# zama-ai/concrete-ntt

Measured on AMD Instinct MI355X. Metric: forward+inverse NTTs/sec (prime64, N=1024, batched) per GPU; % HBM roofline, higher is better.
Workload: dtype u64; 1 GPU; prime64 N=1024 p=4611686018427322369 batch=65536 per GPU: fwd + mul_assign_normalize (pre-transformed rhs) + inv, device-resident, fused in one kernel (cntt_prime64_mul_ntt_batch); polynomial_size=1024, batch_per_gpu=65536, modulus=4611686018427322369, launcher=single process, rccl_ranks=0

## Files before the change

concrete-ntt_amd/csrc/host_core.hip:

```cpp
#include <atomic>
#include <cstdarg>
#include <cstdio>
#include <string>

#include "aux_kernels.hpp"
#include "host_common.hpp"

static thread_local std::string g_err;

int fail(int code, const char *fmt, ...) {
    char buf[512];
    va_list ap;
    va_start(ap, fmt);
    vsnprintf(buf, sizeof buf, fmt, ap);
    va_end(ap);
    g_err = buf;
    return code;
}

extern "C" const char *cntt_last_error(void) { return g_err.c_str(); }
#include "build_hash.inc"
extern "C" const char *cntt_version(void) { return "cntt-hip 0.3 (gfx950) csrc:" CNTT_CSRC_HASH; }
extern "C" int cntt_device_count(void) {
    int n = 0;
    if (hipGetDeviceCount(&n) != hipSuccess) return 0;
    return n;
}

namespace {
struct SwitchDef { const char *name; int dflt; };
constexpr SwitchDef kSwitches[DBG_COUNT] = {
    {"fp", 1}, {"pm64", 1}, {"blk", 1}, {"mul32_blk", 1}, {"ext32_blk", 1}, {"ext_one", 1}, {"ext_split", -1}, {"native_acc", 1},
    {"product_fused", -1}, {"plan52_via32", 1}, {"native_ext", 1}, {"native_gadget", 0}};
std::atomic<int> g_switch[DBG_COUNT] = {{1}, {1}, {1}, {1}, {1}, {1}, {-1}, {1}, {-1}, {1}, {1}, {0}};
int switch_index(const char *key) {
    if (!key) return -1;
    for (int i = 0; i < (int)DBG_COUNT; ++i)
        if (std::strcmp(key, kSwitches[i].name) == 0) return i;
    return -1;
}
}
int cntt::debug_switch(DebugSwitch key) { return g_switch[key].load(std::memory_order_relaxed); }
extern "C" int cntt_debug_set(const char *key, int value) {
    if (key && std::strcmp(key, "reset") == 0) {
        for (int i = 0; i < (int)DBG_COUNT; ++i) g_switch[i].store(kSwitches[i].dflt);
        return CNTT_OK;
    }
    const int i = switch_index(key);
    if (i < 0) return fail(CNTT_EINVAL, "cntt_debug_set: unknown switch '%s'", key ? key : "(null)");
    if (value < -1 || value > 1) return fail(CNTT_EINVAL, "cntt_debug_set: %s takes -1 (library default), 0 or 1", key);
    g_switch[i].store(value < 0 ? kSwitches[i].dflt : value);
    return CNTT_OK;
}
extern "C" int cntt_debug_get(const char *key, int *value) {
    const int i = switch_index(key);
    if (i < 0 || !value) return fail(CNTT_EINVAL, "cntt_debug_get: unknown switch '%s'", key ? key : "(null)");
    *value = g_switch[i].load();
    return CNTT_OK;
}

extern "C" int cntt_shard_bounds(size_t batch, int world, int rank, size_t *begin, size_t *end) {
    if (world < 1 || rank < 0 || rank >= world || !begin || !end) return fail(CNTT_EINVAL, "cntt_shard_bounds: need 0 <= rank < world and non-NULL outputs");
    const size_t base = batch / (size_t)world, rem = batch % (size_t)world, r = (size_t)rank;
    *begin = r * base + (r < rem ? r : rem);
    *end = *begin + base + (r < rem ? 1 : 0);
    return CNTT_OK;
}

extern "C" unsigned cntt_ew_grid(size_t work_items) { return ew_grid(work_items); }

extern "C" int cntt_fill_uniform_u64(uint64_t *dst, size_t count, uint64_t bound, uint64_t seed, void *st) {
    if (!dst && count) return fail(CNTT_EINVAL, "dst is NULL");
    if (!count) return CNTT_OK;
    hipLaunchKernelGGL((fill_uniform_kernel<uint64_t>), dim3(ew_grid(count)), dim3(256), 0, (hipStream_t)st, dst, count,
                       bound, seed);
    HIP_TRY(hipGetLastError());
    return CNTT_OK;
}
extern "C" int cntt_fill_uniform_u32(uint32_t *dst, size_t count, uint32_t bound, uint64_t seed, void *st) {
    if (!dst && count) return fail(CNTT_EINVAL, "dst is NULL");
    if (!count) return CNTT_OK;
    hipLaunchKernelGGL((fill_uniform_kernel<uint32_t>), dim3(ew_grid(count)), dim3(256), 0, (hipStream_t)st, dst, count,
                       bound, seed);
    HIP_TRY(hipGetLastError());
    return CNTT_OK;
}
```

concrete-ntt_amd/csrc/ntt_launch.hpp:

```cpp
#pragma once
#include <hip/hip_runtime.h>
#include <stdint.h>

#include "ntt_arith.hpp"

namespace cntt {
enum DebugSwitch : int {
    DBG_FP = 0,
    DBG_PM64,
    DBG_BLK,
    DBG_MUL32_BLK,
    DBG_EXT32_BLK,
    DBG_EXT_ONE,
    DBG_EXT_SPLIT,
    DBG_NATIVE_ACC,
    DBG_PRODUCT_FUSED,
    DBG_PLAN52_VIA32,
    DBG_NATIVE_EXT,
    DBG_NATIVE_GADGET,
    DBG_COUNT
};
int debug_switch(DebugSwitch key);
}

namespace cntt {

template <class T> struct MaxLdsLogN;
template <> struct MaxLdsLogN<uint64_t> { static constexpr int value = 14; };
template <> struct MaxLdsLogN<uint32_t> { static constexpr int value = 15; };
constexpr int MAX_FPW_LOGN = 15;
template <class T> struct MinLogN;
template <> struct MinLogN<uint64_t> { static constexpr int value = 4; };
template <> struct MinLogN<uint32_t> { static constexpr int value = 5; };

template <class T, bool INV>
hipError_t launch_ntt(int logn, int cls, T *data, const TwPair<T> *tw, const ModParams<T> &P, uint32_t nsub,
                      uint32_t depth, hipStream_t stream);

template <int CLS>
hipError_t launch_ntt_fp(int logn, bool inv, uint64_t *data, const TwPair<uint64_t> *tw, const ModParams<uint64_t> &P,
                         uint32_t nsub, hipStream_t stream);
template <int CLS>
hipError_t launch_mul_ntt_fp(int logn, uint64_t *lhs, const uint64_t *rhs_ntt, const TwPair<uint64_t> *twf,
                             const TwPair<uint64_t> *twi, const ModParams<uint64_t> &P, uint32_t nsub, hipStream_t stream);

template <class T>
hipError_t launch_mul_ntt(int logn, int cls, T *lhs, const T *rhs_ntt, const TwPair<T> *twf, const TwPair<T> *twi,
                          const ModParams<T> &P, uint32_t nsub, hipStream_t stream);

template <class T, int NOUT>
hipError_t launch_ext_ntt_n(int logn, int cls, T *out, const T *terms, const T *key_ntt, const TwPair<T> *twf,
                            const TwPair<T> *twi, const ModParams<T> &P, uint32_t batch, uint32_t nterms, bool accumulate,
                            hipStream_t stream, uint32_t ostride);
bool ext_split_enabled();
template <class T>
inline hipError_t launch_ext_ntt(int logn, int cls, T *out, const T *terms, const T *key_ntt, const TwPair<T> *twf,
                                 const TwPair<T> *twi, const ModParams<T> &P, uint32_t batch, uint32_t nterms, uint32_t nout,
                                 bool accumulate, hipStream_t stream) {
    hipError_t e = hipErrorNotSupported;
    switch (nout) {
    case 0: return hipSuccess;
    case 1: e = launch_ext_ntt_n<T, 1>(logn, cls, out, terms, key_ntt, twf, twi, P, batch, nterms, accumulate, stream, 1); break;
    case 2: e = launch_ext_ntt_n<T, 2>(logn, cls, out, terms, key_ntt, twf, twi, P, batch, nterms, accumulate, stream, 2); break;
    case 3: e = launch_ext_ntt_n<T, 3>(logn, cls, out, terms, key_ntt, twf, twi, P, batch, nterms, accumulate, stream, 3); break;
    case 4: e = launch_ext_ntt_n<T, 4>(logn, cls, out, terms, key_ntt, twf, twi, P, batch, nterms, accumulate, stream, 4); break;
    default: return hipErrorNotSupported;
    }
    if (e != hipErrorNotSupported || nout < 3 || !ext_split_enabled()) return e;
    (void)hipGetLastError();
    e = launch_ext_ntt_n<T, 2>(logn, cls, out, terms, key_ntt, twf, twi, P, batch, nterms, accumulate, stream, nout);
    if (e != hipSuccess) return e;
    T *out2 = out + ((size_t)2 << logn);
    const T *key2 = key_ntt + ((size_t)2 << logn);
    if (nout == 3) return launch_ext_ntt_n<T, 1>(logn, cls, out2, terms, key2, twf, twi, P, batch, nterms, accumulate, stream, nout);
    return launch_ext_ntt_n<T, 2>(logn, cls, out2, terms, key2, twf, twi, P, batch, nterms, accumulate, stream, nout);
}

struct SplitArgs;
struct CrtArgs;
struct AccArgs;
struct ProductArgs;
hipError_t launch_product_fused2(int logn, int cls, bool inv, uint64_t *standard, uint32_t *res32, const void *tables,
                                 const ProductArgs &A, uint32_t batch, bool flag, hipStream_t st);
template <int KIND>
hipError_t launch_native_fused(int logn, void *prod, const void *lhs, const void *rhs, const void *tables, const SplitArgs &S,
                               const CrtArgs &C, uint32_t batch, uint32_t *scratch, hipStream_t st, const AccArgs *acc,
                               const void *tables_acc);
constexpr bool native_fused_acc(int kind, int logn) {
    return kind == 2 ? (logn >= 5 && logn <= 13) : kind == 5 ? (logn >= 5 && logn <= 12) : (kind >= 0 && kind <= 4 && logn >= 5 && logn <= 14);
}
bool native_acc_enabled();
struct KeyPlanes;
constexpr int NATIVE_EXT_MAX_LOGN = 12;
template <int KIND>
hipError_t launch_native_ext(int logn, void *out, const void *terms, const KeyPlanes &K, const void *tables_acc, const SplitArgs &S,
                             const AccArgs &C, uint32_t batch, uint32_t nterms, uint32_t nout, bool accumulate, hipStream_t st);
struct GadgetCall {
    const void *polys;
    const uint32_t *rot;
    const void *addend;
    uint64_t off;
    uint32_t npolys, levels, base_log;
    uint32_t cmux;
    uint32_t add_out;
};
template <int KIND>
hipError_t launch_native_ext_gadget(int logn, void *out, const GadgetCall &G, const KeyPlanes &K, const void *tables_acc,
                                    const SplitArgs &S, const AccArgs &C, uint32_t batch, uint32_t nout, hipStream_t st);
inline int device_num_cus() {
    int dev = 0, n = 0;
    if (hipGetDevice(&dev) != hipSuccess) return 256;
    if (hipDeviceGetAttribute(&n, hipDeviceAttributeMultiprocessorCount, dev) != hipSuccess || n <= 0) n = 256;
    return n;
}
constexpr bool native_fused_lds13(int kind) { return kind == 0 || kind == 1 || kind == 4; }
inline bool native_fused_persistent(int kind, int logn) {
    if (native_fused_acc(kind, logn) && native_acc_enabled()) return false;
    return (logn == 13 && !native_fused_lds13(kind)) || logn == 14 || logn == 15 || (kind == 2 && logn >= 5 && logn <= 12);
}
inline size_t native_fused_tile_words(int logn) { return logn < 12 ? (size_t)4096 : (size_t)1 << logn; }
inline uint32_t native_fused_grid(int logn, int ncu, uint32_t batch) {
    const size_t ppb = native_fused_tile_words(logn) >> logn;
    const size_t groups = ((size_t)batch + ppb - 1) / ppb, g = (size_t)ncu * (logn >= 14 ? 1u : logn == 13 ? 2u : 4u);
    return (uint32_t)(g < groups ? g : groups);
}
inline size_t native_fused_scratch_words(int kind, int logn, int nprimes, int ncu, uint32_t batch) {
    if (!native_fused_persistent(kind, logn)) return 0;
    return (size_t)native_fused_grid(logn, ncu, batch) * (size_t)(nprimes - 1) * native_fused_tile_words(logn);
}

}
```

concrete-ntt_amd/csrc/ntt_mul_inst.inc:

```
#include "ntt_mul_one.hpp"

namespace cntt {

template <class T, int LOGN>
static hipError_t mul_logn(int logn, int cls, T *lhs, const T *rhs, const TwPair<T> *twf, const TwPair<T> *twi,
                           const ModParams<T> &P, uint32_t nsub, hipStream_t stream) {
    if constexpr (sizeof(T) == 4 && LOGN >= 13 && LOGN <= 15) {
        if (logn == LOGN) {
            if constexpr (LOGN >= 14) {
                if (mul32_blk_enabled()) {
                    if constexpr (mul32_blk_wins(LOGN, CLS_FPW)) {
                        if (cls == CLS_FPW) return mul32_blk_one<T, LOGN, CLS_FPW>(lhs, rhs, twf, twi, P, nsub, stream);
                    }
                    if constexpr (mul32_blk_wins(LOGN, CLS_LAZY)) {
                        if (cls == CLS_LAZY) return mul32_blk_one<T, LOGN, CLS_LAZY>(lhs, rhs, twf, twi, P, nsub, stream);
                    }
                    if constexpr (mul32_blk_wins(LOGN, CLS_STRICT)) {
                        if (cls == CLS_STRICT) return mul32_blk_one<T, LOGN, CLS_STRICT>(lhs, rhs, twf, twi, P, nsub, stream);
                    }
                }
            }
            if constexpr (LOGN <= MAX_FPW_LOGN) {
                if (cls == CLS_FPW) {
                    hipLaunchKernelGGL((mul_kernel_one<T, LOGN, CLS_FPW>), dim3(nsub), dim3(MulOne<T, LOGN, CLS_FPW>::TPP), 0, stream, lhs,
                                       rhs, twf, twi, P);
                    return hipGetLastError();
                }
            }
            switch (cls) {
            case CLS_LAZY:
                hipLaunchKernelGGL((mul_kernel_one<T, LOGN, CLS_LAZY>), dim3(nsub), dim3(MulOne<T, LOGN, CLS_LAZY>::TPP), 0, stream, lhs, rhs,
                                   twf, twi, P);
                break;
            case CLS_STRICT:
                hipLaunchKernelGGL((mul_kernel_one<T, LOGN, CLS_STRICT>), dim3(nsub), dim3(MulOne<T, LOGN, CLS_STRICT>::TPP), 0, stream, lhs,
                                   rhs, twf, twi, P);
                break;
            case CLS_GENERIC:
                hipLaunchKernelGGL((mul_kernel_one<T, LOGN, CLS_GENERIC>), dim3(nsub), dim3(MulOne<T, LOGN, CLS_GENERIC>::TPP), 0, stream, lhs,
                                   rhs, twf, twi, P);
                break;
            default: return hipErrorNotSupported;
            }
            return hipGetLastError();
        }
        return mul_logn<T, LOGN + 1>(logn, cls, lhs, rhs, twf, twi, P, nsub, stream);
    } else if constexpr (LOGN > 14) {
        if constexpr (sizeof(T) == 8 && LOGN == 15) {
            if (logn != 15) return hipErrorNotSupported;
            if (cls == CLS_FP) return launch_mul_ntt_fp<CLS_FP>(15, lhs, rhs, twf, twi, P, nsub, stream);
            if (cls == CLS_FP51) return launch_mul_ntt_fp<CLS_FP51>(15, lhs, rhs, twf, twi, P, nsub, stream);
            if (cls == CLS_PM64) return launch_mul_ntt_fp<CLS_PM64>(15, lhs, rhs, twf, twi, P, nsub, stream);
            if (cls == CLS_LAZY) return mul_32k_one<T, CLS_LAZY>(lhs, rhs, twf, twi, P, nsub, stream);
            if (cls == CLS_STRICT) return mul_32k_one<T, CLS_STRICT>(lhs, rhs, twf, twi, P, nsub, stream);
        }
        return hipErrorNotSupported;
    } else {
        using K0 = NttKernel<T, LOGN, false, CLS_LAZY, false>;
        if (logn == LOGN) {
            if constexpr (mul_blk_eligible((int)sizeof(T), LOGN, CLS_LAZY)) {
                if (cls == CLS_FP) return launch_mul_ntt_fp<CLS_FP>(LOGN, lhs, rhs, twf, twi, P, nsub, stream);
                if (cls == CLS_FP51) return launch_mul_ntt_fp<CLS_FP51>(LOGN, lhs, rhs, twf, twi, P, nsub, stream);
                if (cls == CLS_PM64) return launch_mul_ntt_fp<CLS_PM64>(LOGN, lhs, rhs, twf, twi, P, nsub, stream);
                if (cls == CLS_LAZY) return mul_blk_one<T, LOGN, CLS_LAZY>(lhs, rhs, twf, twi, P, nsub, stream);
                if (cls == CLS_STRICT) return mul_blk_one<T, LOGN, CLS_STRICT>(lhs, rhs, twf, twi, P, nsub, stream);
                return hipErrorNotSupported;
            }
            if constexpr (K0::NPASS > 1 && K0::TPP <= 256 && (size_t)K0::IMG_ENTRIES * sizeof(TwPair<T>) <= 32768) {
                if constexpr (sizeof(T) == 8) {
                    if (cls == CLS_FP) return launch_mul_ntt_fp<CLS_FP>(LOGN, lhs, rhs, twf, twi, P, nsub, stream);
                    if (cls == CLS_FP51) return launch_mul_ntt_fp<CLS_FP51>(LOGN, lhs, rhs, twf, twi, P, nsub, stream);
                    if (cls == CLS_PM64) return launch_mul_ntt_fp<CLS_PM64>(LOGN, lhs, rhs, twf, twi, P, nsub, stream);
                }
                if constexpr (sizeof(T) == 4) {
                    if (cls == CLS_FPW) return mul_one<T, LOGN, CLS_FPW>(lhs, rhs, twf, twi, P, nsub, stream);
                }
                switch (cls) {
                case CLS_LAZY: return mul_one<T, LOGN, CLS_LAZY>(lhs, rhs, twf, twi, P, nsub, stream);
                case CLS_STRICT: return mul_one<T, LOGN, CLS_STRICT>(lhs, rhs, twf, twi, P, nsub, stream);
                default: return mul_one<T, LOGN, CLS_GENERIC>(lhs, rhs, twf, twi, P, nsub, stream);
                }
            } else {
                return hipErrorNotSupported;
            }
        }
        return mul_logn<T, LOGN + 1>(logn, cls, lhs, rhs, twf, twi, P, nsub, stream);
    }
}

template <>
hipError_t launch_mul_ntt<INST_T>(int logn, int cls, INST_T *lhs, const INST_T *rhs_ntt, const TwPair<INST_T> *twf,
                                  const TwPair<INST_T> *twi, const ModParams<INST_T> &P, uint32_t nsub,
                                  hipStream_t stream) {
    if (nsub == 0) return hipSuccess;
    if (logn < MinLogN<INST_T>::value || logn > 15) return hipErrorNotSupported;
    return mul_logn<INST_T, MinLogN<INST_T>::value>(logn, cls, lhs, rhs_ntt, twf, twi, P, nsub, stream);
}

}
```

concrete-ntt_amd/csrc/ntt_mul_one.hpp:

```cpp
#pragma once
#include <cstdlib>
#include "ntt_blk.hpp"
#include "ntt_kernel.hpp"
#include "ntt_launch.hpp"

namespace cntt {

template <class T, int LOGN> struct MulShape {
    using K0 = NttKernel<T, LOGN, false, CLS_LAZY, false>;
    static constexpr size_t IMG = (size_t)K0::IMG_ENTRIES * sizeof(TwPair<T>);
    static constexpr size_t LDS_MAX = 160 * 1024;
    static constexpr size_t lds(int block) { return (size_t)(block / K0::TPP) * K0::LDS_WORDS_1 * sizeof(T) + 2 * IMG; }
    static constexpr bool THREE_SMALL = 3 * lds(256) <= LDS_MAX && K0::E == 16;
    static constexpr bool ONE_BIG = !THREE_SMALL && lds(768) <= LDS_MAX && K0::E == 16 && K0::TPP <= 256 && 768 % K0::TPP == 0;
    static constexpr bool TWO_SMALL = 2 * lds(256) <= LDS_MAX;
    static constexpr int BLOCK = THREE_SMALL ? 256 : ONE_BIG ? 768 : TWO_SMALL ? 256 : 512;
    static constexpr int PER_CU = THREE_SMALL ? 3 : ONE_BIG ? 1 : TWO_SMALL ? 2 : 1;
    static constexpr int WAVES_PER_SIMD = BLOCK / 64 * PER_CU / 4;
    static_assert(lds(BLOCK) * PER_CU <= LDS_MAX, "fused product kernel does not fit LDS");
};

static int mul_num_cus() {
    int dev = 0, n = 0;
    if (hipGetDevice(&dev) != hipSuccess) return 256;
    if (hipDeviceGetAttribute(&n, hipDeviceAttributeMultiprocessorCount, dev) != hipSuccess || n <= 0) n = 256;
    return n;
}

template <class T, int LOGN, int CLS>
static hipError_t mul_one(T *lhs, const T *rhs, const TwPair<T> *twf, const TwPair<T> *twi, const ModParams<T> &P,
                          uint32_t nsub, hipStream_t stream) {
    using SH = MulShape<T, LOGN>;
    using K = MulWp<T, LOGN, CLS, SH::BLOCK>;
    const uint32_t ntiles = (nsub + K::PPB - 1) / K::PPB;
    uint32_t grid = (uint32_t)mul_num_cus() * SH::PER_CU;
    if (grid > ntiles) grid = ntiles;
    hipLaunchKernelGGL((mul_kernel_wp<T, LOGN, CLS, SH::BLOCK, SH::WAVES_PER_SIMD>), dim3(grid), dim3(SH::BLOCK), 0, stream,
                       lhs, rhs, twf, twi, P, nsub);
    return hipGetLastError();
}

constexpr bool mul_blk_eligible(int bytes, int logn, int cls) { return bytes == 8 && logn >= 12 && logn <= 14 && cls != CLS_GENERIC; }
template <int LOGN, int CLS> struct MulBlkShape {
    static constexpr int WPW = 4;
    static constexpr int PER_CU = LOGN == 12 ? 4 : LOGN == 13 ? 2 : 1;
    static constexpr bool PREFETCH = true;
    static constexpr int TWC = 2;
};
template <class T, int LOGN, int CLS>
static hipError_t mul_blk_one(T *lhs, const T *rhs, const TwPair<T> *twf, const TwPair<T> *twi, const ModParams<T> &P,
                              uint32_t nsub, hipStream_t stream) {
    using SH = MulBlkShape<LOGN, CLS>;
    using K = MulBlk<T, LOGN, CLS, SH::TWC, SH::PREFETCH>;
    uint32_t grid = (uint32_t)mul_num_cus() * SH::PER_CU;
    if (grid > nsub) grid = nsub;
    hipLaunchKernelGGL((mul_kernel_blk<T, LOGN, CLS, SH::WPW, SH::TWC, SH::PREFETCH>), dim3(grid), dim3(K::WPB), 0, stream, lhs, rhs,
                       twf, twi, P, nsub);
    return hipGetLastError();
}

constexpr bool mul32_blk_wins(int logn, int cls) {
    return (cls == CLS_LAZY && (logn == 14 || logn == 15)) || (cls == CLS_STRICT && logn == 15) || (cls == CLS_FPW && logn == 14);
}
static bool mul32_blk_enabled() { return debug_switch(DBG_MUL32_BLK) != 0; }
template <class T, int LOGN, int CLS>
static hipError_t mul32_blk_one(T *lhs, const T *rhs, const TwPair<T> *twf, const TwPair<T> *twi, const ModParams<T> &P,
                                uint32_t nsub, hipStream_t stream) {
    constexpr bool PF = LOGN == 14 && CLS == CLS_LAZY;
    using K = MulBlk<T, LOGN, CLS, 2, PF>;
    uint32_t grid = (uint32_t)mul_num_cus() * (LOGN == 14 ? 2 : 1);
    if (grid > nsub) grid = nsub;
    hipLaunchKernelGGL((mul_kernel_blk<T, LOGN, CLS, 4, 2, PF>), dim3(grid), dim3(K::WPB), 0, stream, lhs, rhs, twf, twi, P, nsub);
    return hipGetLastError();
}

template <class T, int CLS>
static hipError_t mul_32k_one(T *lhs, const T *rhs, const TwPair<T> *twf, const TwPair<T> *twi, const ModParams<T> &P,
                              uint32_t nsub, hipStream_t stream) {
    uint32_t grid = (uint32_t)mul_num_cus();
    if (grid > nsub) grid = nsub;
    hipLaunchKernelGGL((mul_kernel_32k<T, CLS, 4>), dim3(grid), dim3(Mul32k<T, CLS>::WPB), 0, stream, lhs, rhs, twf, twi, P, nsub);
    return hipGetLastError();
}

}
```

Baseline: 239.8 million NTT/s.

## Add paired-polynomial wavefront kernel for fused N=1024 multiply NTT

Adds a new fused forward-multiply-inverse kernel for 64-bit lazy-class N=1024 in which each wavefront transforms two polynomials at once. Twiddle loads, stage bookkeeping and the per-wave LDS buffer are shared across the pair. The next tile's two polynomials are prefetched asynchronously while the current tile is computed. The kernel is enabled by default through a new mul_pair switch. In exchange it doubles register pressure per thread and serialises the LDS transposes for the two polynomials, which may lower occupancy.

```diff
diff --git a/concrete-ntt_amd/csrc/host_core.hip b/concrete-ntt_amd/csrc/host_core.hip
--- a/concrete-ntt_amd/csrc/host_core.hip
+++ b/concrete-ntt_amd/csrc/host_core.hip
@@ -31,8 +31,8 @@
 struct SwitchDef { const char *name; int dflt; };
 constexpr SwitchDef kSwitches[DBG_COUNT] = {
     {"fp", 1}, {"pm64", 1}, {"blk", 1}, {"mul32_blk", 1}, {"ext32_blk", 1}, {"ext_one", 1}, {"ext_split", -1}, {"native_acc", 1},
-    {"product_fused", -1}, {"plan52_via32", 1}, {"native_ext", 1}, {"native_gadget", 0}};
-std::atomic<int> g_switch[DBG_COUNT] = {{1}, {1}, {1}, {1}, {1}, {1}, {-1}, {1}, {-1}, {1}, {1}, {0}};
+    {"product_fused", -1}, {"plan52_via32", 1}, {"native_ext", 1}, {"native_gadget", 0}, {"mul_pair", 1}};
+std::atomic<int> g_switch[DBG_COUNT] = {{1}, {1}, {1}, {1}, {1}, {1}, {-1}, {1}, {-1}, {1}, {1}, {0}, {1}};
 int switch_index(const char *key) {
     if (!key) return -1;
     for (int i = 0; i < (int)DBG_COUNT; ++i)
diff --git a/concrete-ntt_amd/csrc/ntt_launch.hpp b/concrete-ntt_amd/csrc/ntt_launch.hpp
--- a/concrete-ntt_amd/csrc/ntt_launch.hpp
+++ b/concrete-ntt_amd/csrc/ntt_launch.hpp
@@ -18,6 +18,7 @@
     DBG_PLAN52_VIA32,
     DBG_NATIVE_EXT,
     DBG_NATIVE_GADGET,
+    DBG_MUL_PAIR,
     DBG_COUNT
 };
 int debug_switch(DebugSwitch key);
diff --git a/concrete-ntt_amd/csrc/ntt_mul_inst.inc b/concrete-ntt_amd/csrc/ntt_mul_inst.inc
--- a/concrete-ntt_amd/csrc/ntt_mul_inst.inc
+++ b/concrete-ntt_amd/csrc/ntt_mul_inst.inc
@@ -75,6 +75,9 @@
                 if constexpr (sizeof(T) == 4) {
                     if (cls == CLS_FPW) return mul_one<T, LOGN, CLS_FPW>(lhs, rhs, twf, twi, P, nsub, stream);
                 }
+                if constexpr (mul_pair_eligible((int)sizeof(T), LOGN, CLS_LAZY)) {
+                    if (cls == CLS_LAZY && mul_pair_enabled()) return mul_pair_one<T, LOGN, CLS_LAZY>(lhs, rhs, twf, twi, P, nsub, stream);
+                }
                 switch (cls) {
                 case CLS_LAZY: return mul_one<T, LOGN, CLS_LAZY>(lhs, rhs, twf, twi, P, nsub, stream);
                 case CLS_STRICT: return mul_one<T, LOGN, CLS_STRICT>(lhs, rhs, twf, twi, P, nsub, stream);
diff --git a/concrete-ntt_amd/csrc/ntt_mul_one.hpp b/concrete-ntt_amd/csrc/ntt_mul_one.hpp
--- a/concrete-ntt_amd/csrc/ntt_mul_one.hpp
+++ b/concrete-ntt_amd/csrc/ntt_mul_one.hpp
@@ -3,6 +3,7 @@
 #include "ntt_blk.hpp"
 #include "ntt_kernel.hpp"
 #include "ntt_launch.hpp"
+#include "ntt_mul_pair.hpp"
 
 namespace cntt {
 
@@ -37,6 +38,23 @@
     if (grid > ntiles) grid = ntiles;
     hipLaunchKernelGGL((mul_kernel_wp<T, LOGN, CLS, SH::BLOCK, SH::WAVES_PER_SIMD>), dim3(grid), dim3(SH::BLOCK), 0, stream,
                        lhs, rhs, twf, twi, P, nsub);
+    return hipGetLastError();
+}
+
+constexpr bool mul_pair_eligible(int bytes, int logn, int cls) { return bytes == 8 && logn == 10 && cls == CLS_LAZY; }
+static bool mul_pair_enabled() { return debug_switch(DBG_MUL_PAIR) != 0; }
+template <class T, int LOGN, int CLS>
+static hipError_t mul_pair_one(T *lhs, const T *rhs, const TwPair<T> *twf, const TwPair<T> *twi, const ModParams<T> &P,
+                               uint32_t nsub, hipStream_t stream) {
+    constexpr int BLOCK = 256, PER_CU = 2, WAVES_PER_SIMD = BLOCK / 64 * PER_CU / 4;
+    using K = MulWpPair<T, LOGN, CLS, BLOCK>;
+    static_assert(PER_CU * ((size_t)(BLOCK / K::TPP) * K::FB::LDS_WORDS_1 * sizeof(T) + 2 * MulShape<T, LOGN>::IMG) <= MulShape<T, LOGN>::LDS_MAX,
+                  "pair kernel does not fit LDS");
+    const uint32_t ntiles = (nsub + K::PPB - 1) / K::PPB;
+    uint32_t grid = (uint32_t)mul_num_cus() * PER_CU;
+    if (grid > ntiles) grid = ntiles;
+    hipLaunchKernelGGL((mul_kernel_wp_pair<T, LOGN, CLS, BLOCK, WAVES_PER_SIMD>), dim3(grid), dim3(BLOCK), 0, stream, lhs, rhs, twf, twi,
+                       P, nsub);
     return hipGetLastError();
 }
 
diff --git a/concrete-ntt_amd/csrc/ntt_mul_pair.hpp b/concrete-ntt_amd/csrc/ntt_mul_pair.hpp
--- /dev/null
+++ b/concrete-ntt_amd/csrc/ntt_mul_pair.hpp
@@ -0,0 +1,200 @@
+#pragma once
+#include "ntt_kernel.hpp"
+
+namespace cntt {
+
+template <class T, int LOGN, int CLS, int WPB>
+struct MulWpPair {
+    using F = NttWp<T, LOGN, false, CLS, WPB>;
+    using I = NttWp<T, LOGN, true, CLS, WPB>;
+    using FB = typename F::B;
+    using IB = typename I::B;
+    template <bool INV> using KB = std::conditional_t<INV, IB, FB>;
+    static constexpr int E = FB::E, LOGE = FB::LOGE, TPP = FB::TPP, NPASS = FB::NPASS;
+    static constexpr int PPW = 2;
+    static constexpr int PPB = PPW * (WPB / TPP);
+    static constexpr uint32_t FULL = FB::FULL;
+    static constexpr uint32_t RM0 = FB::S::RMASK[0], RMM = FB::S::RMASK[NPASS - 1], RML = IB::S::RMASK[NPASS - 1];
+    static constexpr uint32_t IO_RM = F::IO_RM;
+    static constexpr int NV = E / FB::MAXV;
+    static_assert(RMM == IB::S::RMASK[0], "forward and inverse schedules must mirror each other");
+    static_assert(TPP == 64 && FB::WAVE_PRIVATE, "a wavefront owns whole polynomials");
+    static_assert(RM0 == IO_RM && RML == IO_RM, "the first and last register layouts are the coalesced one");
+    static_assert(NV == 8, "wait_pair ties sixteen vectors");
+    static_assert(!BoxOps<CLS>::template USE<T>::value && !Bfly<T, CLS>::IS_FP, "integer butterflies on plain words");
+
+    template <bool INV, int K, int GI>
+    static __device__ __forceinline__ void stage(T (&r0)[E], T (&r1)[E], uint32_t ebase, const TwPair<T> *__restrict__ tw,
+                                                 const ModParams<T> &P, uint32_t tid, const TwPair<T> *img) {
+        using NB = KB<INV>;
+        using S = typename NB::S;
+        constexpr uint32_t RM = S::RMASK[K], GM = S::GMASK[K], CM = FULL & ~RM;
+        constexpr int b = NB::nth_stage_bit(GM, GI), k = crank(RM, b), NHI = 1 << (LOGE - 1 - k);
+        if constexpr (INV && b == LOGN - 1) {
+#pragma unroll
+            for (int j = 0; j < E; ++j) {
+                if ((j >> k) & 1) continue;
+                Bfly<T, CLS>::inv_norm(r0[j], r0[j | (1 << k)], P);
+                Bfly<T, CLS>::inv_norm(r1[j], r1[j | (1 << k)], P);
+            }
+            return;
+        }
+        uint32_t toff = 1u << (LOGN - 1 - b);
+        if constexpr ((CM >> (b + 1)) != 0u) toff += ebase >> (b + 1);
+        constexpr typename NB::StageGeom g = NB::geom(K, GI);
+        constexpr bool UNI = g.uniform;
+        constexpr bool FIRST = !INV && NB::stage_no(K, GI) == 0;
+        TwPair<T> w[NHI];
+#pragma unroll
+        for (int h = 0; h < NHI; ++h) {
+            if constexpr (!g.uniform) w[h] = img[NB::img_off(K, GI) + h * g.d + (tid >> g.shift)];
+            else w[h] = NB::tw_at(tw, toff, cdep((uint32_t)h << (k + 1), RM) >> (b + 1));
+        }
+#pragma unroll
+        for (int j = 0; j < E; ++j) {
+            if ((j >> k) & 1) continue;
+            const int h = j >> (k + 1);
+            if constexpr (INV) {
+                Bfly<T, CLS>::template inv<UNI>(r0[j], r0[j | (1 << k)], w[h].w, w[h].ws, P);
+                Bfly<T, CLS>::template inv<UNI>(r1[j], r1[j | (1 << k)], w[h].w, w[h].ws, P);
+            } else {
+                Bfly<T, CLS>::template fwd<UNI, FIRST>(r0[j], r0[j | (1 << k)], w[h].w, w[h].ws, P);
+                Bfly<T, CLS>::template fwd<UNI, FIRST>(r1[j], r1[j | (1 << k)], w[h].w, w[h].ws, P);
+            }
+        }
+    }
+    template <bool INV, int K, int GI = 0>
+    static __device__ __forceinline__ void stages(T (&r0)[E], T (&r1)[E], uint32_t ebase, const TwPair<T> *__restrict__ tw,
+                                                  const ModParams<T> &P, uint32_t tid, const TwPair<T> *img) {
+        if constexpr (GI < cpop(KB<INV>::S::GMASK[K])) {
+            stage<INV, K, GI>(r0, r1, ebase, tw, P, tid, img);
+            stages<INV, K, GI + 1>(r0, r1, ebase, tw, P, tid, img);
+        }
+    }
+    template <bool INV, bool FIN, int K = 0>
+    static __device__ __forceinline__ void pass(T (&r0)[E], T (&r1)[E], T *lds, uint32_t tid, const TwPair<T> *__restrict__ tw,
+                                                const TwPair<T> *img, const ModParams<T> &P) {
+        using NB = KB<INV>;
+        constexpr uint32_t RM = NB::S::RMASK[K];
+        const uint32_t ebase = pdep<FULL & ~RM>(tid);
+        stages<INV, K>(r0, r1, ebase, tw, P, tid, img);
+        if constexpr (K < NPASS - 1) {
+            constexpr uint32_t RMN = NB::S::RMASK[K + 1];
+            const uint32_t ebn = pdep<FULL & ~RMN>(tid);
+            NB::sync();
+            NB::template scatter<RM>(r0, lds, ebase, true);
+            NB::sync();
+            NB::template gather<RMN>(r0, (const T *)lds, ebn, true);
+            NB::sync();
+            NB::template scatter<RM>(r1, lds, ebase, true);
+            NB::sync();
+            NB::template gather<RMN>(r1, (const T *)lds, ebn, true);
+            pass<INV, FIN, K + 1>(r0, r1, lds, tid, tw, img, P);
+        } else if constexpr (FIN) {
+#pragma unroll
+            for (int j = 0; j < E; ++j) {
+                r0[j] = INV ? Bfly<T, CLS>::finish_inv(r0[j], P) : Bfly<T, CLS>::finish_fwd(r0[j], P);
+                r1[j] = INV ? Bfly<T, CLS>::finish_inv(r1[j], P) : Bfly<T, CLS>::finish_fwd(r1[j], P);
+            }
+        }
+    }
+
+    using AsyncVec = typename FB::AsyncVec;
+    template <int YOUNGER> static __device__ __forceinline__ void wait_pair(AsyncVec (&a)[NV], AsyncVec (&b)[NV]) {
+        asm volatile("s_waitcnt vmcnt(%16)"
+                     : "+v"(a[0]), "+v"(a[1]), "+v"(a[2]), "+v"(a[3]), "+v"(a[4]), "+v"(a[5]), "+v"(a[6]), "+v"(a[7]),
+                       "+v"(b[0]), "+v"(b[1]), "+v"(b[2]), "+v"(b[3]), "+v"(b[4]), "+v"(b[5]), "+v"(b[6]), "+v"(b[7])
+                     : "n"(YOUNGER)
+                     : "memory");
+    }
+
+    static __device__ __forceinline__ void run(T *__restrict__ lhs, const T *__restrict__ rhs_ntt,
+                                               const TwPair<T> *__restrict__ twf, const TwPair<T> *__restrict__ twi,
+                                               const ModParams<T> &P, uint32_t nsub, T *lds_all, TwPair<T> *imgf,
+                                               TwPair<T> *imgi) {
+        FB::fill_image(imgf, twf);
+        IB::fill_image(imgi, twi);
+        __syncthreads();
+        const ModParams<T> Pi = mul_inv_params<T, CLS>(P);
+        const uint32_t tid = threadIdx.x & (TPP - 1);
+        const uint32_t wv = threadIdx.x / TPP;
+        const uint32_t pl = wv * PPW;
+        T *lds = lds_all + (size_t)wv * FB::LDS_WORDS_1;
+        constexpr uint32_t CMM = FULL & ~RMM, CMIO = FULL & ~IO_RM;
+        const uint32_t ebaseM = pdep<CMM>(tid), ebaseIO = pdep<CMIO>(tid);
+        const uint32_t ntiles = (nsub + PPB - 1) / PPB;
+        const uint32_t voffIO = ((pl << LOGN) + ebaseIO) * (uint32_t)sizeof(T);
+        constexpr uint32_t POLY_BYTES = (uint32_t)sizeof(T) << LOGN;
+        T r0[E], r1[E];
+#pragma unroll
+        for (int j = 0; j < E; ++j) r0[j] = r1[j] = 0;
+        uint32_t tile = blockIdx.x;
+        if (tile < ntiles) {
+            const uint32_t last = nsub - 1u - tile * PPB;
+            const uint32_t c0 = pl < last ? pl : last, c1 = pl + 1u < last ? pl + 1u : last;
+            const T *tb = (const T *)(lhs + (((size_t)tile * PPB) << LOGN));
+            AsyncVec v0[NV], v1[NV];
+            FB::template gather_async<IO_RM>(v0, tb, ((c0 << LOGN) + ebaseIO) * (uint32_t)sizeof(T));
+            FB::template gather_async<IO_RM>(v1, tb, ((c1 << LOGN) + ebaseIO) * (uint32_t)sizeof(T));
+            wait_pair<0>(v0, v1);
+            FB::unpack_async(r0, v0);
+            FB::unpack_async(r1, v1);
+        }
+        constexpr int NST = PPW * (E / FB::template vec_elems<IO_RM>());
+        for (; tile < ntiles; tile += gridDim.x) {
+            const uint32_t sub = tile * PPB + pl;
+            const uint32_t tnext = tile + gridDim.x;
+            const bool more = tnext < ntiles;
+            T *tbase = lhs + (((size_t)tile * PPB) << LOGN);
+            AsyncVec vn0[NV], vn1[NV];
+            if (more) {
+                const uint32_t last = nsub - 1u - tnext * PPB;
+                const uint32_t c0 = pl < last ? pl : last, c1 = pl + 1u < last ? pl + 1u : last;
+                const T *tb = (const T *)(lhs + (((size_t)tnext * PPB) << LOGN));
+                FB::template gather_async<IO_RM>(vn0, tb, ((c0 << LOGN) + ebaseIO) * (uint32_t)sizeof(T));
+                FB::template gather_async<IO_RM>(vn1, tb, ((c1 << LOGN) + ebaseIO) * (uint32_t)sizeof(T));
+            }
+#pragma unroll
+            for (int j = 0; j < E; ++j) {
+                r0[j] = Bfly<T, CLS>::load_fix(r0[j], P);
+                r1[j] = Bfly<T, CLS>::load_fix(r1[j], P);
+            }
+            pass<false, mul_fwd_fin<T, CLS>()>(r0, r1, lds, tid, twf, imgf, P);
+            {
+                const uint32_t lastc = nsub - 1u - tile * PPB;
+                const uint32_t c0 = pl < lastc ? pl : lastc, c1 = pl + 1u < lastc ? pl + 1u : lastc;
+                const T *rb = rhs_ntt + (((size_t)tile * PPB) << LOGN);
+                T b[E];
+                FB::template gather_tile<RMM>(b, rb, ((c0 << LOGN) + ebaseM) * (uint32_t)sizeof(T));
+#pragma unroll
+                for (int j = 0; j < E; ++j) r0[j] = mul_fused<T, CLS>(r0[j], b[j], P);
+                FB::template gather_tile<RMM>(b, rb, ((c1 << LOGN) + ebaseM) * (uint32_t)sizeof(T));
+#pragma unroll
+                for (int j = 0; j < E; ++j) r1[j] = mul_fused<T, CLS>(r1[j], b[j], P);
+            }
+            pass<true, true>(r0, r1, lds, tid, twi, imgi, Pi);
+            if (sub < nsub) FB::template scatter_tile<IO_RM>(r0, tbase, voffIO);
+            if (sub + 1u < nsub) FB::template scatter_tile<IO_RM>(r1, tbase, voffIO + POLY_BYTES);
+            FB::sync();
+            if (more) {
+                wait_pair<NST>(vn0, vn1);
+                FB::unpack_async(r0, vn0);
+                FB::unpack_async(r1, vn1);
+            }
+        }
+    }
+};
+
+template <class T, int LOGN, int CLS, int WPB, int WPW>
+__global__ __launch_bounds__(WPB, WPW) void mul_kernel_wp_pair(T *__restrict__ lhs, const T *__restrict__ rhs_ntt,
+                                                           const TwPair<T> *__restrict__ twf,
+                                                           const TwPair<T> *__restrict__ twi, const ModParams<T> P,
+                                                           uint32_t nsub) {
+    using K = MulWpPair<T, LOGN, CLS, WPB>;
+    __shared__ __attribute__((aligned(16))) T lds[(size_t)(WPB / K::TPP) * K::FB::LDS_WORDS_1];
+    __shared__ __attribute__((aligned(16))) TwPair<T> imgf[K::FB::IMG_ENTRIES];
+    __shared__ __attribute__((aligned(16))) TwPair<T> imgi[K::IB::IMG_ENTRIES];
+    K::run(lhs, rhs_ntt, twf, twi, P, nsub, lds, imgf, imgi);
+}
+
+}
```

Measured after the change: 238.4 million NTT/s. Within noise of the previous version (-0.6%).
